# rusty-shell/rust-compress

Measured on AMD Instinct MI355X. Metric: GiB/s decoded output (batched blocks), higher is better.
Workload: dtype u8; 1 GPU; LZ4 block decode, 4096 independent 64 KiB blocks per GPU (BASELINE configs[1]); distribution=G-text, kernel_variant=0, parallelism=blocks sharded, 4096 per rank, no collective

## Files before the change

rust_compress_amd/csrc/k_lz4_decode_v8.hip:

```cpp
#include "rcx_dev.h"
#include "k_lz4_emit6.hip"

#ifndef RCX_V8_PSLEEP
#define RCX_V8_PSLEEP 16
#endif
#ifndef RCX_V8_ESLEEP
#define RCX_V8_ESLEEP 2
#endif
#ifndef RCX_FIELDS_ISA
#define RCX_FIELDS_ISA 1
#endif
#ifndef RCX_WALK_FORM
#define RCX_WALK_FORM 5
#endif
#ifndef RCX_V8_PRE
#define RCX_V8_PRE 128
#endif
#ifndef RCX_LINK_REPAIR
#define RCX_LINK_REPAIR 1
#endif
#ifndef RCX_WALK_STEPS
#define RCX_WALK_STEPS 16
#endif
#ifndef RCX_WALK_ISA_LOW
// ... 738 lines not shown
            const int agev = (agey ? 1 : 0) | ((RCX_AGE_LOW && (tail & 3u) < ((uint32_t)(RCX_AGE_LOW >> (4u * agerank)) & 15u)) ? 2 : 0);
            tail++;
            if (lane == 0) ring->tail = tail;
            if (X6 && plain6) { RCX_V8_STAT(10, lane == 0 && bt.why == B::SOLO_); RCX_V8_STAT(11, lane == 0 && bt.why == B::WIDE_); RCX_V8_STAT(12, lane == 0 ? (uint32_t)bt.ns : 0u); RCX_V8_STAT(13, lane == 0); }
            if (X6 && plain6 && this->emit6(bt.ns, w1, p0, agev)) {
                if (this->after_batch(bt, st)) break;
                continue;
            }
            RCX_V8_STAT(9, lane == 0 && bt.ns > 0);
            RCX_V8_STAT(10, lane == 0 && bt.why == B::SOLO_); RCX_V8_STAT(11, lane == 0 && bt.why == B::WIDE_); RCX_V8_STAT(12, lane == 0 ? (uint32_t)bt.ns : 0u); RCX_V8_STAT(13, lane == 0);
            const bool cont = (w1 & 0x80u) != 0;
            if (cont) w1 &= ~0xffu;
            const uint32_t L = w1 & 0xffu, M = (w1 >> 8) & 0xffu;
            const uint32_t hop = ((int)lane < bt.ns && !cont) ? 3u + L + (L >= 15u ? 1u : 0u) + (M >= 19u ? 1u : 0u) : 0u;
            const uint32_t w0 = p0 + rcx_wave_incl_scan(hop) - hop + 1u + (L >= 15u ? 1u : 0u);
            int lo = 0, e = 0;
            RCX_MARK("x8_pre_emit");
            if (PROF8) { const uint64_t t_ = (uint64_t)__builtin_readcyclecounter(); this->pw[1] += t_ - te1; te1 = t_; }
#if defined(RCX_DUMMY_SALU) || defined(RCX_DUMMY_VALU) || defined(RCX_DUMMY_VCMP) || defined(RCX_DUMMY_VCMPX) || defined(RCX_DUMMY_RL) || defined(RCX_DUMMY_SNOP) || defined(RCX_DUMMY_BR) || defined(RCX_DUMMY_LDS)
            {
                uint32_t ds_ = 0, dv_ = this->lane;
#ifdef RCX_DUMMY_SALU
#pragma unroll
                for (int k_ = 0; k_ < RCX_DUMMY_SALU; k_++) asm volatile("s_add_u32 %0, %0, 1" : "+s"(ds_) : : "scc");
#endif
#ifdef RCX_DUMMY_VALU
#pragma unroll
                for (int k_ = 0; k_ < RCX_DUMMY_VALU; k_++) asm volatile("v_add_u32_e32 %0, 1, %0" : "+v"(dv_));
#endif
#ifdef RCX_DUMMY_VCMP
#pragma unroll
                for (int k_ = 0; k_ < RCX_DUMMY_VCMP; k_++) asm volatile("v_cmp_lt_u32_e32 vcc, %0, %0" : : "v"(dv_) : "vcc");
#endif
#ifdef RCX_DUMMY_VCMPX
#pragma unroll
                for (int k_ = 0; k_ < RCX_DUMMY_VCMPX; k_++) asm volatile("v_cmpx_le_u32_e32 vcc, %0, %0" : : "v"(dv_) : "vcc");
#endif
#ifdef RCX_DUMMY_RL
#pragma unroll
                for (int k_ = 0; k_ < RCX_DUMMY_RL; k_++) asm volatile("v_readlane_b32 %0, %1, 0" : "=s"(ds_) : "v"(dv_));
#endif
#ifdef RCX_DUMMY_SNOP
#pragma unroll
                for (int k_ = 0; k_ < RCX_DUMMY_SNOP; k_++) asm volatile("s_nop 0");
#endif
#ifdef RCX_DUMMY_BR
#pragma unroll
                for (int k_ = 0; k_ < RCX_DUMMY_BR; k_++) asm volatile("s_cbranch_execz 1f\n1:");
#endif
#ifdef RCX_DUMMY_LDS
#pragma unroll
                for (int k_ = 0; k_ < RCX_DUMMY_LDS; k_++) asm volatile("ds_read_b32 %0, %1" : "=v"(dv_) : "v"(0u) : "memory");
                asm volatile("s_waitcnt lgkmcnt(0)" ::: "memory");
#endif
                asm volatile("" : : "s"(ds_), "v"(dv_));
            }
#endif
            if (CUT & 8) { if (!(CUT & 32)) this->oend += RCX_U(__builtin_amdgcn_readlane(w0, 63)) & 1u; lo = bt.ns; if (bt.why == B::END_ || bt.why == B::ERR_) break; continue; }
            while (lo < bt.ns && !e) e = this->template emit5<false, PRED, CUT, (SPLIT ? SPLIT : 64), typename std::conditional<X6, Lz4V8, void>::type>(bt.ns, lo, w0, w1, nullptr, agev);
            RCX_MARK("x8_post_emit");
            if (e) { st = e; break; }
            if (PROF8) te1 = (uint64_t)__builtin_readcyclecounter();
            if (this->after_batch(bt, st)) break;
            if (PROF8) this->pw[3] += (uint64_t)__builtin_readcyclecounter() - te1;
            RCX_MARK("x8_loop_end");
        }
        if (st && lane == 0) ring->abort_ = 1;
        if (RCX_AGE_DYN && lane == 0) __hip_atomic_store(prog + wslot, RCX_PROG_FIN, __ATOMIC_RELAXED, __HIP_MEMORY_SCOPE_AGENT);
        if (!st) this->flush(this->oend, true);
        *st_out = st;
        *len_out = st ? 0u : this->oend;
    }

    __device__ void run_parser8()
    {
        this->lane = rcx_lane();
        const unsigned lane = this->lane;
        const uint32_t n = this->n;
        const uint32_t inmis = (uint32_t)((uintptr_t)this->in & 15u);
        uint32_t head = 0;
        uint32_t c = 0;
        int32_t cs = -(int32_t)inmis;
        uint32_t lcnt = 0;
        while (c < n) {
            V8P_T0();
            if (RCX_V8_ADAPT) ring_prio(head, RCX_V8_LOW_WALK);
            else if (c != 0 && RCX_WALK_PRIO != RCX_PARSER_PRIO) __builtin_amdgcn_s_setprio(RCX_WALK_PRIO);
            else if ((RCX_AGE_PRIO & 16) && this->agey) __builtin_amdgcn_s_setprio(RCX_PARSER_PRIO + 1); else __builtin_amdgcn_s_setprio(RCX_PARSER_PRIO);
            stage8(cs);
#if RCX_V8_PREFETCH
            {
                const int64_t q = (int64_t)cs + CH + CSLACK + 64 * (int64_t)lane;
                if (q >= 0 && q + 4 <= (int64_t)n) { const uint32_t x = *(const rcx_u32_u*)(this->in + q); asm volatile("" : : "v"(x)); }
            }
#endif
            const int nseg = ((int64_t)n - cs >= CH) ? NSEG : (int)(((int64_t)n - cs + SEGB - 1) / SEGB);
            const int k0 = (int)(((int32_t)c - cs) / SEGB);
            const int32_t s = cs + SEGB * (int32_t)lane;
            const uint32_t e = ((int64_t)s + SEGB < (int64_t)n) ? (uint32_t)(s + SEGB) : n;
            const uint32_t nx = RCX_U(next_tok_c(c));
            const bool giant = nx >= n || (int64_t)nx >= (int64_t)cs + CH;
            const bool mine = !giant && (int)lane >= k0 && (int)lane < nseg;
            int32_t p0 = s - PRE; p0 = p0 < 0 ? 0 : p0;
            uint32_t p = ((int)lane == k0) ? c : (uint32_t)p0;
            uint64_t map = (giant && (int)lane == k0) ? 1ull << (c - (uint32_t)s) : 0ull;
            RCX_MARK("p8_walk");
#if (RCX_WALK_FORM == 5) && !defined(RCX_NO_WALK_ASM)
            if (n >= 20u) {
                const uint32_t adj = RCX_U((uint32_t)(uintptr_t)this->cbuf - (uint32_t)this->cbase);
                const uint32_t e20 = e < n - 19u ? e : n - 19u;
                const uint32_t ead = mine ? e20 + adj : 0u, sgad = (uint32_t)s + adj;
                uint32_t ad = p + adj;
                for (;;) {
                    uint32_t steps = RCX_WALK_STEPS;
                    const uint64_t slow = walk_steps2(ad, ead, sgad, map, steps);
                    if (PROF8) pp[7] += steps == 0xffffffffu ? 0 : RCX_WALK_STEPS - steps;
                    if (slow) { if (RCX_INV_BALLOT(slow)) ad = next_tok(ad - adj) + adj; }
                    else if (steps == 0xffffffffu) break;
                    if (RCX_V8_ADAPT) ring_prio(head, RCX_V8_LOW_WALK);
                }
                p = ad - adj; p = p < n ? p : n;
            }
#elif (RCX_WALK_FORM >= 2) && !defined(RCX_NO_WALK_ASM)
            if (n >= 20u && (RCX_WALK_FORM == 2 || head == 0 || (RCX_WALK_FORM == 4 && head - RCX_U(this->ring8->tail) < (uint32_t)RCX_WALK_ISA_LOW))) {
                uint32_t mlo = (uint32_t)map, mhi = (uint32_t)(map >> 32);
                const uint64_t minem = __ballot(mine);
                for (;;) {
                    uint32_t steps = 4;
                    const uint64_t slow = walk_steps(p, e, (uint32_t)s, mlo, mhi, minem, steps);
                    if (PROF8) pp[7] += steps == 0xffffffffu ? 0 : 4 - steps;
                    if (slow) { if (RCX_INV_BALLOT(slow)) p = next_tok(p); }
                    else if (steps == 0xffffffffu) break;
                    if (RCX_V8_ADAPT) ring_prio(head, RCX_V8_LOW_WALK);
                }
                map = (uint64_t)mlo | ((uint64_t)mhi << 32);
            } else
#endif
            for (uint32_t wstep = 0;; wstep++) {
                const bool go = mine && p < e;
                if (!__ballot(go)) break;
                if (PROF8) pp[7] += 1;
                if (RCX_V8_ADAPT && (wstep & 3u) == 3u) ring_prio(head, RCX_V8_LOW_WALK);
#if RCX_WALK_FORM == 0 || RCX_WALK_FORM >= 3
                if (go) {
                    if ((int32_t)p >= s) map |= 1ull << (p - (uint32_t)s);
                    p = next_tok_c(p);
                }
#else
                const uint32_t q = next_tok_c(p, go);
                const uint64_t bit = (go && (int32_t)p >= s) ? 1ull << ((p - (uint32_t)s) & 63u) : 0ull;
                map |= bit;
                p = go ? q : p;
#endif
            }
            RCX_MARK("p8_walk_end");
            const uint32_t ex = p;
            V8P_ADD(0);
            if (RCX_V8_ADAPT) ring_prio(head, RCX_V8_LOW_WALK);
            uint32_t lowv = 0; bool clr = false;
            if (giant) c = nx;
            else {
                const uint32_t eprev = (uint32_t)__shfl_up((int)ex, 1);
                const bool chk = mine && (int)lane > k0;
                bool ok = false;
                if (chk && eprev < e) { lowv = eprev - (uint32_t)s; ok = (map >> lowv) & 1ull; }
                if (!ok) lowv = 0;
                unsigned long long bad = __ballot(chk && !ok);
#ifdef RCX_LINK_NOREPAIR
                bad = 0;
#endif
                c = RCX_U(__builtin_amdgcn_readlane(ex, nseg - 1));
                int k = 0; uint32_t cin = 0; bool forced = false;
                for (;;) {
                    if (!forced) {
                        if (!bad) break;
                        k = __ffsll(bad) - 1;
                        cin = RCX_U(__builtin_amdgcn_readlane(ex, k - 1));
                    }
                    bad &= ~(1ull << k);
                    const uint32_t sk = (uint32_t)(cs + SEGB * k);
                    const uint32_t ek = (sk + SEGB < n) ? sk + SEGB : n;
                    const uint32_t exk = RCX_U(__builtin_amdgcn_readlane(ex, k));
                    uint32_t X;
                    if (cin >= ek) { if ((int)lane == k) { clr = true; lowv = 0; } X = cin; }
                    else {
                        const uint64_t mk = (uint64_t)RCX_U(__builtin_amdgcn_readlane((uint32_t)map, k)) | ((uint64_t)RCX_U(__builtin_amdgcn_readlane((uint32_t)(map >> 32), k)) << 32);
                        if ((mk >> (cin - sk)) & 1ull) { if ((int)lane == k) { lowv = cin - sk; clr = false; } X = exk; }
                        else {
                            if (PROF8) pp[8] += 1;
                            uint64_t tm = 0;
                            uint32_t q = cin;
#if RCX_LINK_REPAIR
                            {
                                const int32_t qi = (int32_t)(sk + lane) - this->cbase;
                                const uint32_t t = ((const RCX_LDS_AS uint8_t*)this->cbuf)[qi];
                                const uint32_t L = t >> 4;
                                const uint32_t x = ((const RCX_LDS_AS uint8_t*)this->cbuf)[qi + 3 + (int32_t)L];
                                const bool ext = (t & 15u) == 15u;
                                const bool fastp = n >= 20u && sk + lane <= n - 20u && L != 15u && !(ext && x == 255u);
                                const uint32_t dv = fastp ? (ext ? 4u : 3u) + L : 128u;
                                uint32_t rel = cin - sk;
                                RCX_V8_STAT(7, lane == 0);
                                for (;;) {
                                    uint64_t vis = 0;
                                    RCX_HOP_WALK(dv, rel, vis);
                                    tm |= vis;
                                    RCX_V8_STAT(7, lane == 0 ? (uint64_t)__popcll(vis) << 32 : 0ull); RCX_V8_STAT(19, lane == 0 && rel >= 128u);
                                    if (rel < 128u) { q = sk + rel; break; }
                                    q = RCX_U(next_tok_c(sk + rel - 128u));
                                    if (q >= ek) break;
                                    rel = q - sk;
                                }
                            }
                            if ((int)lane == k) { map = tm; lowv = 0; clr = false; }
                            X = q;
#else
                            while (q < ek && !((mk >> (q - sk)) & 1ull)) { tm |= 1ull << (q - sk); q = RCX_U(next_tok_c(q)); }
                            const bool merged = q < ek;
                            const uint64_t nm = (merged ? mk & ~((1ull << (q - sk)) - 1ull) : 0ull) | tm;
                            if ((int)lane == k) { map = nm; lowv = 0; clr = false; }
                            X = merged ? exk : q;
#endif
                        }
                    }
                    if (k == nseg - 1) c = X;
                    forced = X != exk && k + 1 < nseg;
                    if (forced) { k++; cin = X; }
                }
            }
            if (clr) map = 0;
            map &= ~((1ull << lowv) - 1ull);
            if (!mine && !giant) map = 0;
            V8P_ADD(1);
            RCX_MARK("p8_link_end");
            if (PROF8) pp[6] += 1;
            const int nwin = (nseg + LWIN - 1) / LWIN;
            for (int w = k0 / LWIN; w < nwin; w++) {
                if (RCX_V8_ADAPT) ring_prio(head);
                const int sl = LWIN * w + (int)(lane >> 3);
                const uint32_t mlo = (uint32_t)__builtin_amdgcn_ds_bpermute(sl << 2, (int)(uint32_t)map);
                const uint32_t mhi = (uint32_t)__builtin_amdgcn_ds_bpermute(sl << 2, (int)(uint32_t)(map >> 32));
                uint32_t bits = (((lane & 4u) ? mhi : mlo) >> (8u * (lane & 3u))) & 0xffu;
                if (sl >= nseg) bits = 0;
                const uint32_t cnt = (uint32_t)__popc(bits);
                const uint32_t incl = rcx_wave_incl_scan(cnt);
                uint32_t at = lcnt + incl - cnt;
                const int32_t bpos = SEGB * sl + 8 * (int32_t)(lane & 7u);
                for (;;) {
                    if (!__ballot(bits != 0)) break;
                    if (bits) { const uint32_t b = (uint32_t)__ffs(bits) - 1u; bits &= bits - 1u; list[at++] = (int16_t)(bpos + (int32_t)b); }
                }
                lcnt += RCX_U(__builtin_amdgcn_readlane(incl, 63));
                rcx_wave_sync();
                V8P_ADD(2);
                RCX_MARK("p8_list_end");
                const bool last = (w + 1 == nwin) && c >= n;
                uint32_t pos = 0;
                while (lcnt - pos >= 64u || (last && lcnt > pos)) {
                    const int used = batch8(head, cs, pos, lcnt - pos < 64u ? lcnt - pos : 64u);
                    if (used < 0) return;
                    pos += (uint32_t)used;
                    if (PROF8) t0_ = (uint64_t)__builtin_readcyclecounter();
                }
                if (pos) {
                    const uint32_t left = lcnt - pos;
                    const int16_t v = lane < left ? list[pos + lane] : (int16_t)0;
                    rcx_wave_sync();
                    if (lane < left) list[lane] = v;
                    lcnt = left;
                    rcx_wave_sync();
                }
            }
            int32_t ncs = cs + CH;
            if (c < n && (int64_t)c >= (int64_t)ncs + CH) ncs = (int32_t)((c + inmis) & ~15u) - (int32_t)inmis;
            if (lcnt) {
                if ((int32_t)(int16_t)RCX_U((uint32_t)(uint16_t)list[0]) - (ncs - cs) < -30000) {
                    uint32_t pos = 0;
                    while (lcnt > pos) { const int used = batch8(head, cs, pos, lcnt - pos); if (used < 0) return; pos += (uint32_t)used; }
                    lcnt = 0;
                } else {
                    if (lane < lcnt) list[lane] = (int16_t)(list[lane] - (int16_t)(ncs - cs));
                    rcx_wave_sync();
                }
            }
            cs = ncs;
        }
        post(head, 0, B::END_, 0, 0, 0, 0, 0, 0, false, 0, 0, 0);
    }
};

template <int TC = 1024, int HH = 768, bool PROF8 = false, int PRE_ = RCX_V8_PRE, int SPLIT_ = 32, bool PRED = false, int PRR = 2, int CUT = 0, bool MIRROR = false, int X6_ = -1>
__global__ __launch_bounds__(128, 8) void k_lz4_decode_v8(rcx_kargs a, int only_status = 0)
{
    constexpr bool X6 = RCX_X6_MODE != 0 && (X6_ < 0 ? (CUT == 0 && !PRED && SPLIT_ != 0 && !MIRROR) : X6_ != 0);
    typedef Lz4V8<TC, HH, X6 ? 0 : 16, PROF8, PRE_, SPLIT_, PRED, PRR, CUT, MIRROR, X6> S;
    __shared__ __align__(16) uint32_t s_mtab[X6 ? 20 * RCX_X6_MROW : 4];
    const uint64_t tk0 = PROF8 ? (uint64_t)__builtin_readcyclecounter() : 0;
    const uint64_t rt0 = PROF8 ? (uint64_t)__builtin_amdgcn_s_memrealtime() : 0;
    __shared__ __align__(16) uint8_t s_wbuf[S::WBUF5 + 16 + (X6 ? 16 : 0)];
    __shared__ __align__(16) typename S::Ring8 s_ring;
    __shared__ __align__(16) uint8_t s_cbuf[S::CBUF8 + 16];
    __shared__ int16_t s_list[S::LISTN];
    __shared__ uint32_t s_lmap[64];
    const uint32_t b = blockIdx.x;
    if (b >= a.nblocks) return;
    if (only_status && a.status[b] != only_status) return;
    if (MIRROR && a.gate) {
        uint32_t r = 0;
#pragma unroll
        for (int i = 0; i < 15; i++) r += b >= a.gate_bnd[i] ? 1u : 0u;
        if (r || a.gate_all) {
            if (threadIdx.x == 0) {
                const uint64_t t0 = __builtin_amdgcn_s_memrealtime();
                uint32_t ok = 1;
                if (b == (r ? a.gate_bnd[r - 1] : 0u)) {
                    while (__hip_atomic_load(a.gate_host + r, __ATOMIC_RELAXED, __HIP_MEMORY_SCOPE_SYSTEM) != a.gate_seq) {
                        __builtin_amdgcn_s_sleep(60);
                        if (__builtin_amdgcn_s_memrealtime() - t0 > (uint64_t)a.gate_ticks) { ok = 0; break; }
                    }
                    if (ok) __hip_atomic_store(a.gate + r, a.gate_seq, __ATOMIC_RELEASE, __HIP_MEMORY_SCOPE_SYSTEM);
                }
                while (ok && __hip_atomic_load(a.gate + r, __ATOMIC_RELAXED, __HIP_MEMORY_SCOPE_SYSTEM) != a.gate_seq) {
                    __builtin_amdgcn_s_sleep(127); __builtin_amdgcn_s_sleep(127);
                    if (__builtin_amdgcn_s_memrealtime() - t0 > (uint64_t)a.gate_ticks) ok = 0;
                }
                s_lmap[0] = ok;
            }
            __syncthreads();
            const uint32_t ok = s_lmap[0];
            __builtin_amdgcn_fence(__ATOMIC_ACQUIRE, "");
            __syncthreads();
            if (!ok) { if (threadIdx.x == 0) a.status[b] = (int32_t)RCX_ST_GATE; return; }
        }
    }
    if (threadIdx.x == 0) { RCX_LDS_AS typename S::Ring8* r0 = (RCX_LDS_AS typename S::Ring8*)&s_ring; r0->head = 0; r0->tail = 0; r0->abort_ = 0; }
    __syncthreads();
    const uint32_t role = (uint32_t)__builtin_amdgcn_readfirstlane((int)(threadIdx.x >> 6));
    S s;
    s.in = a.in_base + a.in_off[b];
    s.n = (uint32_t)a.in_len[b];
    s.out = a.out_base + a.out_off[b];
    if (MIRROR) s.out2 = a.out_mirror + a.out_off[b];
    const uint64_t cap64 = a.out_cap[b];
    s.cap = cap64 > 0xffffffffull ? 0xffffffffu : (uint32_t)cap64;
    s.cbuf = s_cbuf;
    s.wb_ = s_wbuf + (X6 ? 16 : 0);
    s.epos = nullptr;
    s.ring = nullptr;
    s.ring8 = (RCX_LDS_AS typename S::Ring8*)&s_ring;
    s.list = s_list;
    s.lmap = s_lmap;
    s.mtab = (RCX_LDS_AS uint32_t*)s_mtab;
    if (RCX_AGE_DYN) {
        const uint32_t hw = (uint32_t)__builtin_amdgcn_s_getreg((15 << 11) | (0 << 6) | 4);
        const uint32_t xcc = (uint32_t)__builtin_amdgcn_s_getreg((3 << 11) | (0 << 6) | 20) & 15u;
        s.prog = g_lz4_prog + 8u * (((hw >> 4) & 0xfffu) | (xcc << 12));
        s.wslot = hw & 7u;
    }
    if (role == 0) {
        if (RCX_AGE_DYN && (threadIdx.x & 63u) == 0) __hip_atomic_store(s.prog + s.wslot, RCX_PROG_PARSER, __ATOMIC_RELAXED, __HIP_MEMORY_SCOPE_AGENT);
        if (RCX_AGE_PRIO & 16) s.agey = (((uint32_t)__builtin_amdgcn_s_getreg((3 << 11) | (0 << 6) | 4) >> 1) & 7u) >= (uint32_t)RCX_AGE_SPLIT;
        s.run_parser8();
        if (PROF8 && a.scratch && (threadIdx.x & 63u) == 0) {
            uint64_t* q = (uint64_t*)a.scratch + (size_t)b * 32;
            for (int i = 0; i < 10; i++) q[i] = s.pp[i];
            q[10] = (uint64_t)__builtin_readcyclecounter() - tk0;
        }
        return;
    }
    int32_t st; uint32_t olen;
    const uint32_t hwid = (PROF8 || RCX_AGE_PRIO) ? (uint32_t)__builtin_amdgcn_s_getreg((3 << 11) | (0 << 6) | 4) : 0u;
    s.agey = RCX_AGE_PRIO ? ((hwid >> 1) & 7u) >= (uint32_t)RCX_AGE_SPLIT : true;
    s.agerank = (hwid >> 1) & 3u;
    RCX_SETPRIO_EXEC(s.agey);
    if (X6) { s.lane = rcx_lane(); s.mtab_init(); }
    s.run_executor8(&st, &olen);
    if (PROF8 && a.scratch && (threadIdx.x & 63u) == 0) {
        uint64_t* q = (uint64_t*)a.scratch + (size_t)b * 32;
        q[11] = (uint64_t)__builtin_readcyclecounter() - tk0;
        q[12] = hwid;
        q[13] = rt0; q[14] = (uint64_t)__builtin_amdgcn_s_memrealtime();
        q[15] = (uint64_t)(uint32_t)__builtin_amdgcn_s_getreg((31 << 11) | (0 << 6) | 4) | ((uint64_t)(uint32_t)__builtin_amdgcn_s_getreg((31 << 11) | (0 << 6) | 20) << 32);
        for (int i = 0; i < 12; i++) q[16 + i] = s.pw[i];
    }
    if ((threadIdx.x & 63u) == 0) {
        a.status[b] = st;
        a.out_len[b] = olen;
        if (a.in_used) a.in_used[b] = s.n;
    }
}
```

rust_compress_amd/csrc/k_lz4_emit6.hip:

```cpp
#pragma once
#include "rcx_dev.h"

#ifndef RCX_X6_MROW
#define RCX_X6_MROW 9
#endif
#ifndef RCX_X6_RR
#define RCX_X6_RR 3
#endif
#ifndef RCX_X6_MODE
#define RCX_X6_MODE 1
#endif
#ifndef RCX_X6_ROUNDS_ASM
#define RCX_X6_ROUNDS_ASM 1
#endif
#ifndef RCX_X6_EARLY
#define RCX_X6_EARLY 1
#endif
#ifndef RCX_V8_STAT
#define RCX_V8_STAT(slot, v) ((void)0)
#endif

#if !defined(RCX_NO_ROUNDS_ASM) && !defined(RCX_NO_MSKOR_ASM)
__device__ __forceinline__ uint64_t rcx_lz4_rounds6(uint32_t s0, uint32_t d4, uint32_t mc, uint32_t dep_lo, uint32_t dep_hi, uint64_t pend, uint32_t tb, uint32_t fix)
{
    uint32_t t0, t1, nv, sa, sh, da, r0, r1, r2, r3, r4, r5, m0, m1, m2, m3, m4, prog = 0;
    uint64_t sT, sF;
    asm volatile(
        "s_mov_b64 vcc, %[pend]\n\t"
        "L_top_%=:\n\t"
        "v_and_b32_e32 %[t0], vcc_lo, %[dlo]\n\t"
        "v_and_b32_e32 %[t1], vcc_hi, %[dhi]\n\t"
        "v_or_b32_e32 %[t0], %[t0], %[t1]\n\t"
        "v_cmp_eq_u32_e64 %[sT], 0, %[t0]\n\t"
        "s_and_b64 exec, %[sT], vcc\n\t"
        "s_cbranch_scc0 L_out_%=\n\t"
        "v_add_u32_e32 %[sa], %[s0], %[prog]\n\t"
        "v_sub_u32_e32 %[nv], %[mc], %[prog]\n\t"
        "v_and_b32_e32 %[t0], -4, %[sa]\n\t"
        "ds_read_b32 %[r0], %[t0]\n\t"
        "ds_read_b32 %[r1], %[t0] offset:4\n\t"
        "ds_read_b32 %[r2], %[t0] offset:8\n\t"
        "ds_read_b32 %[r3], %[t0] offset:12\n\t"
        "ds_read_b32 %[r4], %[t0] offset:16\n\t"
        "ds_read_b32 %[r5], %[t0] offset:20\n\t"
        "v_min_u32_e32 %[nv], 16, %[nv]\n\t"
        "v_mad_u32_u24 %[t1], %[nv], %[mrow], %[tb]\n\t"
        "ds_read_b32 %[m0], %[t1]\n\t"
        "ds_read_b32 %[m1], %[t1] offset:4\n\t"
        "ds_read_b32 %[m2], %[t1] offset:8\n\t"
        "ds_read_b32 %[m3], %[t1] offset:12\n\t"
        "ds_read_b32 %[m4], %[t1] offset:16\n\t"
        "v_and_b32_e32 %[sh], 3, %[sa]\n\t"
        "v_add_u32_e32 %[da], %[d4], %[prog]\n\t"
        "v_add_u32_e32 %[prog], %[prog], %[nv]\n\t"
        "v_cmp_ge_u32_e64 %[sF], %[prog], %[mc]\n\t"
        "s_waitcnt lgkmcnt(9)\n\t"
        "v_alignbyte_b32 %[r0], %[r1], %[r0], %[sh]\n\t"
        "s_waitcnt lgkmcnt(8)\n\t"
        "v_alignbyte_b32 %[r1], %[r2], %[r1], %[sh]\n\t"
        "s_waitcnt lgkmcnt(7)\n\t"
        "v_alignbyte_b32 %[r2], %[r3], %[r2], %[sh]\n\t"
        "s_waitcnt lgkmcnt(6)\n\t"
        "v_alignbyte_b32 %[r3], %[r4], %[r3], %[sh]\n\t"
        "s_waitcnt lgkmcnt(5)\n\t"
        "v_alignbyte_b32 %[r4], %[r5], %[r4], %[sh]\n\t"
        "s_waitcnt lgkmcnt(4)\n\t"
        "v_and_b32_e32 %[m0], %[m0], %[fix]\n\t"
        "v_and_b32_e32 %[r0], %[r0], %[m0]\n\t"
        "ds_mskor_b32 %[da], %[m0], %[r0]\n\t"
        "s_waitcnt lgkmcnt(4)\n\t"
        "v_and_b32_e32 %[r1], %[r1], %[m1]\n\t"
        "ds_mskor_b32 %[da], %[m1], %[r1] offset:4\n\t"
        "s_waitcnt lgkmcnt(4)\n\t"
        "v_and_b32_e32 %[r2], %[r2], %[m2]\n\t"
        "ds_mskor_b32 %[da], %[m2], %[r2] offset:8\n\t"
        "s_waitcnt lgkmcnt(4)\n\t"
        "v_and_b32_e32 %[r3], %[r3], %[m3]\n\t"
        "ds_mskor_b32 %[da], %[m3], %[r3] offset:12\n\t"
        "s_waitcnt lgkmcnt(4)\n\t"
        "v_and_b32_e32 %[r4], %[r4], %[m4]\n\t"
        "ds_mskor_b32 %[da], %[m4], %[r4] offset:16\n\t"
        "s_mov_b64 exec, -1\n\t"
        "s_andn2_b64 vcc, vcc, %[sF]\n\t"
        "s_cbranch_scc1 L_top_%=\n\t"
        "L_out_%=:\n\t"
        "s_mov_b64 exec, -1\n\t"
        "s_mov_b64 %[pend], vcc\n\t"
        : [pend] "+s"(pend), [prog] "+v"(prog), [t0] "=&v"(t0), [t1] "=&v"(t1), [nv] "=&v"(nv), [sa] "=&v"(sa), [sh] "=&v"(sh), [da] "=&v"(da),
          [r0] "=&v"(r0), [r1] "=&v"(r1), [r2] "=&v"(r2), [r3] "=&v"(r3), [r4] "=&v"(r4), [r5] "=&v"(r5),
          [m0] "=&v"(m0), [m1] "=&v"(m1), [m2] "=&v"(m2), [m3] "=&v"(m3), [m4] "=&v"(m4), [sT] "=&s"(sT), [sF] "=&s"(sF)
        : [s0] "v"(s0), [d4] "v"(d4), [mc] "v"(mc), [dlo] "v"(dep_lo), [dhi] "v"(dep_hi), [tb] "v"(tb), [fix] "v"(fix), [mrow] "s"(4u * (uint32_t)RCX_X6_MROW)
        : "vcc", "scc", "memory");
    return pend;
}
#define RCX_HAVE_ROUNDS6 1
#endif

template <class Base, bool PROF8>
struct Lz4X6 : Base {
    typedef Base P5;
    typedef typename Base::B B;
    RCX_LDS_AS uint32_t* mtab = nullptr;

    __device__ __forceinline__ void mtab_init()
    {
        for (uint32_t i = this->lane; i < 20u * (uint32_t)RCX_X6_MROW; i += 64u) {
            const int32_t e = (int32_t)(i / (uint32_t)RCX_X6_MROW), k = (int32_t)(i % (uint32_t)RCX_X6_MROW);
            int32_t t = e - 4 * k; t = t < 0 ? 0 : t > 4 ? 4 : t;
            mtab[i] = (k < 5 && t) ? (0xffffffffu >> (8 * (4 - t))) : 0u;
        }
        rcx_wave_sync();
    }
    template <int NW>
    __device__ __forceinline__ void store_frame(uint8_t* fp, uint32_t w0, uint32_t w1, uint32_t w2, uint32_t w3, uint32_t w4, uint32_t a, uint32_t n)
    {
#ifdef RCX_NO_MSKOR_ASM
        const uint32_t w[5] = {w0, w1, w2, w3, w4};
        for (uint32_t j = a; j < a + n; j++) fp[j] = (uint8_t)(w[j >> 2] >> (8u * (j & 3u)));
#else
        const RCX_LDS_AS uint32_t* te = mtab + (uint32_t)RCX_X6_MROW * (a + n);
#if RCX_X6_MROW == 8
        const rcx_u32x4 mv = *(const RCX_LDS_AS rcx_u32x4*)te;
#else
        rcx_u32x4 mv; mv[0] = te[0]; mv[1] = te[1]; mv[2] = te[2]; mv[3] = te[3];
#endif
        const uint32_t m0 = mv[0] & (0xffffffffu << (8u * a));
        const uint32_t fa = (uint32_t)(uintptr_t)fp;
        if (NW >= 5) {
            const uint32_t m4 = te[4];
            asm volatile("ds_mskor_b32 %0, %1, %2\n\tds_mskor_b32 %0, %3, %4 offset:4\n\tds_mskor_b32 %0, %5, %6 offset:8\n\tds_mskor_b32 %0, %7, %8 offset:12\n\tds_mskor_b32 %0, %9, %10 offset:16"
                         :: "v"(fa), "v"(m0), "v"(w0 & m0), "v"(mv[1]), "v"(w1 & mv[1]), "v"(mv[2]), "v"(w2 & mv[2]), "v"(mv[3]), "v"(w3 & mv[3]), "v"(m4), "v"(w4 & m4) : "memory");
        } else {
            asm volatile("ds_mskor_b32 %0, %1, %2\n\tds_mskor_b32 %0, %3, %4 offset:4\n\tds_mskor_b32 %0, %5, %6 offset:8\n\tds_mskor_b32 %0, %7, %8 offset:12"
                         :: "v"(fa), "v"(m0), "v"(w0 & m0), "v"(mv[1]), "v"(w1 & mv[1]), "v"(mv[2]), "v"(w2 & mv[2]), "v"(mv[3]), "v"(w3 & mv[3]) : "memory");
        }
#endif
    }

    __device__ __forceinline__ bool emit6(int ns, uint32_t w1raw, uint32_t p0, int young)
    {
        const unsigned lane = this->lane;
        const uint8_t* in = this->in; uint8_t* out = this->out; uint8_t* wb_ = this->wb_;
        const uint32_t cap = this->cap, n = this->n;
        uint64_t tq_ = PROF8 ? (uint64_t)__builtin_readcyclecounter() : 0;
#define X6P_ADD(slot) do { RCX_MARK("emit6_" #slot); if (PROF8) { const uint64_t t1_ = (uint64_t)__builtin_readcyclecounter(); this->pw[slot] += t1_ - tq_; tq_ = t1_; } } while (0)
        this->make_room(B::TCAP);
        X6P_ADD(11);
        const uint32_t oend0 = this->oend;
        const uint32_t w1 = (int)lane < ns ? w1raw : 0u;
        const uint32_t L = w1 & 0x7fu, M = (w1 >> 8) & 0xffu, off = w1 >> 16;
        const uint32_t lx = L >= 15u ? 1u : 0u;
        const uint32_t hop = ((int)lane < ns && !(w1 & 0x80u)) ? 3u + L + lx + (M >= 19u ? 1u : 0u) : 0u;
        const uint32_t len = L + M;
        const uint32_t sc = rcx_wave_incl_scan(len | (hop << 16));
        const uint32_t T = RCX_U(__builtin_amdgcn_readlane(sc, 63)) & 0xffffu;
        if (T > (uint32_t)B::TCAP || cap - oend0 < T + 64u) return false;
        const uint32_t lincl = sc & 0xffffu;
        const uint32_t ostart = oend0 + lincl - len;
        const uint32_t mdst = ostart + L;
        const uint32_t src = p0 + (sc >> 16) - hop + 1u + lx;
        const uint32_t slo = mdst - off;
        const uint32_t re = this->rlo_eff();
        const bool isfar = slo < re;
        if (__ballot(off > mdst || (isfar && slo < 4u))) return false;
        X6P_ADD(4);

        const int32_t lbase = this->lbase;
        const int32_t li_o = (int32_t)ostart - lbase, li_m = li_o + (int32_t)L;
        const uint32_t a1 = (uint32_t)li_o & 3u, a2 = (uint32_t)li_m & 3u;
        uint32_t ql = src - a1; { const uint32_t qm = n - 36u; ql = ql < qm ? ql : qm; }
        const bool lit2 = __ballot(L > 16u) != 0;
        const rcx_u32x4 g0 = *(const rcx_u32x4_u*)(in + ql);
        const rcx_u32x4 g1 = *(const rcx_u32x4_u*)(in + ql + 16);
        uint32_t g2 = 0;
        if (lit2) g2 = *(const rcx_u32_u*)(in + ql + 32);
        rcx_u32x4 f0, f1; uint32_t f2;
        RCX_NOINIT4(f0); RCX_NOINIT4(f1); f2 = 0;
#ifndef RCX_X6_NOFAR
        if (re) {
#else
        if (false) {
#endif
            const uint32_t qf = isfar ? slo - a2 : 0u;
            f0 = *(const rcx_u32x4_u*)(out + qf);
            f1 = *(const rcx_u32x4_u*)(out + qf + 16);
            f2 = *(const rcx_u32_u*)(out + qf + 32);
        }
        RCX_SETPRIO_ROUND(young);

        const uint32_t shi = (slo + M < mdst) ? slo + M : mdst;
        bool inb = M != 0u && !isfar && shi > oend0;
        uint32_t S = off;
        uint32_t ka, kb;
        {
            uint32_t* const lmap = this->lmap;
            uint8_t* const lcnt = (uint8_t*)(lmap + P5::LMW);
            lmap[lane] = 0;
            rcx_wave_sync();
            const uint32_t rel = lincl - len;
            atomicOr(&lmap[rel >> 5], 1u << (rel & 31u));
            rcx_wave_sync();
            const uint32_t pc = (uint32_t)__popc(lmap[lane]);
            const uint32_t ex = rcx_wave_incl_scan(pc) - pc;
            lcnt[lane] = (uint8_t)ex;
            rcx_wave_sync();
            int32_t ra = (int32_t)(slo - oend0), rb = (int32_t)(shi - oend0) - 1;
            ra = ra > 0 ? ra : 0; rb = rb > 0 ? rb : 0;
            uint32_t ca = lcnt[ra >> 5], ma = lmap[ra >> 5], cb2 = lcnt[rb >> 5], mb = lmap[rb >> 5];
            RCX_SETTLE4(ca, ma, cb2, mb);
            ka = (ca + (uint32_t)__popc(ma & (0xffffffffu >> (31u - ((uint32_t)ra & 31u)))) - 1u) & 63u;
            kb = (cb2 + (uint32_t)__popc(mb & (0xffffffffu >> (31u - ((uint32_t)rb & 31u)))) - 1u) & 63u;
        }
        unsigned long long dep = 0;
        {
            const uint32_t pmd = (uint32_t)__builtin_amdgcn_ds_bpermute((int)(ka << 2), (int)((isfar || off < M) ? 0xffffffffu : mdst));
            const uint32_t prod = (inb && ka == kb && slo >= pmd && off >= M) ? ka : 64u;
            RCX_V8_STAT(28, inb && ka != kb); RCX_V8_STAT(29, inb && ka == kb && slo < pmd); RCX_V8_STAT(30, inb && ka == kb && slo >= pmd && off < M);
            RCX_V8_STAT(31, inb && ka == kb && shi <= pmd && pmd != 0xffffffffu);
            uint32_t st = prod | (ka << 7) | (kb << 13) | ((uint32_t)inb << 19);
#pragma unroll
            for (int rr = 0; rr < RCX_X6_RR; rr++) {
                const bool has = (st & 64u) == 0u;
                const uint32_t j = has ? (st & 63u) : lane;
                const uint32_t Sj = (uint32_t)__builtin_amdgcn_ds_bpermute((int)(j << 2), (int)S);
                const uint32_t pk = (uint32_t)__builtin_amdgcn_ds_bpermute((int)(j << 2), (int)st);
                const uint32_t Sn = S + Sj;
                const bool ok = has && mdst - Sn >= re && Sn <= mdst;
                S = ok ? Sn : S;
                st = ok ? pk : (st | 64u);
            }
            ka = (st >> 7) & 63u; kb = (st >> 13) & 63u; inb = (st >> 19) & 1u;
            const unsigned long long upto = (kb >= 63) ? ~0ull : ((2ull << kb) - 1ull);
            dep = inb ? (upto & ~((1ull << ka) - 1ull) & ((1ull << lane) - 1ull)) : 0ull;
        }

        X6P_ADD(5);
        {
            const uint32_t n1 = L < 16u ? L : 16u;
            uint8_t* fp = wb_ + (li_o - (int32_t)a1);
            if (n1) store_frame<5>(fp, g0[0], g0[1], g0[2], g0[3], g1[0], a1, n1);
            if (lit2) { if (L > 16u) store_frame<5>(fp + 16, g1[0], g1[1], g1[2], g1[3], g2, a1, L - n1); }
        }
#if RCX_X6_EARLY
        const bool early = M != 0u && !isfar && !inb && off >= M && (RCX_X6_EARLY == 1 || M <= 16u);
        RCX_V8_STAT(15, early);
        if (early) {
            const int32_t sb = (int32_t)(mdst - S) - lbase - (int32_t)a2;
#ifdef RCX_NO_MSKOR_ASM
            const RCX_LDS_AS uint32_t* q = (const RCX_LDS_AS uint32_t*)(wb_ + (sb & ~3));
#else
            uint32_t qa = (uint32_t)(uintptr_t)wb_ + (uint32_t)(sb & ~3);
            asm volatile("" : "+v"(qa));
            const RCX_LDS_AS uint32_t* q = (const RCX_LDS_AS uint32_t*)qa;
#endif
            const uint32_t sh = (uint32_t)sb & 3u;
            const uint32_t r0 = q[0], r1 = q[1], r2 = q[2], r3 = q[3], r4 = q[4], r5 = q[5];
            f0[0] = RCX_ALIGNBYTE(r1, r0, sh); f0[1] = RCX_ALIGNBYTE(r2, r1, sh); f0[2] = RCX_ALIGNBYTE(r3, r2, sh); f0[3] = RCX_ALIGNBYTE(r4, r3, sh);
            f1[0] = RCX_ALIGNBYTE(r5, r4, sh);
            if (RCX_X6_EARLY == 1 && M > 16u) {
                const uint32_t r6 = q[6], r7 = q[7], r8 = q[8], r9 = q[9];
                f1[1] = RCX_ALIGNBYTE(r6, r5, sh); f1[2] = RCX_ALIGNBYTE(r7, r6, sh); f1[3] = RCX_ALIGNBYTE(r8, r7, sh); f2 = RCX_ALIGNBYTE(r9, r8, sh);
            }
        }
        const uint32_t mf = (isfar || early) ? M : 0u;
        if (__ballot(mf != 0u)) {
#else
        const uint32_t mf = isfar ? M : 0u;
        if (re) {
#endif
            const uint32_t n1 = mf < 16u ? mf : 16u;
            uint8_t* fp = wb_ + (li_m - (int32_t)a2);
            if (n1) store_frame<5>(fp, f0[0], f0[1], f0[2], f0[3], f1[0], a2, n1);
            if (mf > 16u) store_frame<5>(fp + 16, f1[0], f1[1], f1[2], f1[3], f2, a2, mf - n1);
        }
        rcx_wave_sync();
        X6P_ADD(6);

        {
            const int32_t dfr = li_m - (int32_t)a2;
            const bool ovl = M != 0u && off < 16u && off < M;
            const int32_t sfr = isfar ? dfr : (int32_t)(mdst - S) - lbase - (int32_t)a2;
            const uint32_t Mc = mf ? 0u : M;
            auto fill_run = [&]() __attribute__((always_inline)) {
                uint32_t done = 0, back = off;
                while (done < M) {
                    uint32_t c = back < M - done ? back : M - done;
                    c = c < 16u ? c : 16u;
                    const int32_t d = li_m + (int32_t)done;
                    const uint32_t ar = (uint32_t)d & 3u;
                    const int32_t sb = d - (int32_t)back - (int32_t)ar;
                    const uint32_t* q = (const uint32_t*)(wb_ + (sb & ~3));
                    const uint32_t sh = (uint32_t)sb & 3u;
                    const uint32_t r0 = q[0], r1 = q[1], r2 = q[2], r3 = q[3], r4 = q[4], r5 = q[5];
                    store_frame<5>(wb_ + (d - (int32_t)ar), RCX_ALIGNBYTE(r1, r0, sh), RCX_ALIGNBYTE(r2, r1, sh), RCX_ALIGNBYTE(r3, r2, sh),
                                   RCX_ALIGNBYTE(r4, r3, sh), RCX_ALIGNBYTE(r5, r4, sh), ar, c);
                    done += c;
                    if (2u * back <= off + done) back *= 2u;
                }
            };
            unsigned long long pm = __ballot(Mc != 0u);
#ifdef RCX_HAVE_ROUNDS6
            if (RCX_X6_ROUNDS_ASM) {
                const uint32_t wa = (uint32_t)(uintptr_t)wb_;
                const unsigned long long depx = dep | (ovl ? 1ull << lane : 0ull);
                while (pm) {
                    pm = rcx_lz4_rounds6(wa + (uint32_t)sfr, wa + (uint32_t)dfr, Mc, (uint32_t)depx, (uint32_t)(depx >> 32), pm,
                                         (uint32_t)(uintptr_t)mtab + a2 * (4u * (uint32_t)RCX_X6_MROW), 0xffffffffu << (8u * a2));
                    if (!pm) break;
                    const bool fill = ovl && ((pm >> lane) & 1ull) && (pm & dep) == 0ull;
                    if (fill) fill_run();
                    rcx_wave_sync();
                    pm &= ~__ballot(fill);
                }
            } else
#endif
            {
            uint32_t prog = 0;
            RCX_V8_STAT(16, Mc != 0u); RCX_V8_STAT(17, Mc != 0u && dep != 0ull); RCX_V8_STAT(18, Mc > 16u);
            uint32_t nr_ = 0;
            while (pm) {
                nr_++; RCX_V8_STAT(14, lane == 0);
                const bool ready = ((pm >> lane) & 1ull) && (pm & dep) == 0ull;
                const bool fill = ready && ovl;
                const uint32_t left = Mc - prog;
                const uint32_t nv = (ready && !ovl) ? (left < 16u ? left : 16u) : 0u;
                const int32_t sb = sfr + (int32_t)prog;
                const uint32_t* q = (const uint32_t*)(wb_ + (sb & ~3));
                const uint32_t sh = (uint32_t)sb & 3u;
                uint32_t r0 = 0, r1 = 0, r2 = 0, r3 = 0, r4 = 0, r5 = 0;
                if (nv) { r0 = q[0]; r1 = q[1]; r2 = q[2]; r3 = q[3]; r4 = q[4]; r5 = q[5]; }
                rcx_wave_sync();
                if (nv) store_frame<5>(wb_ + (dfr + (int32_t)prog), RCX_ALIGNBYTE(r1, r0, sh), RCX_ALIGNBYTE(r2, r1, sh), RCX_ALIGNBYTE(r3, r2, sh),
                               RCX_ALIGNBYTE(r4, r3, sh), RCX_ALIGNBYTE(r5, r4, sh), a2, nv);
                if (fill) fill_run();
                rcx_wave_sync();
                prog += fill ? Mc : nv;
                pm = __ballot(prog < Mc);
            }
            RCX_V8_STAT(20 + (nr_ < 7u ? nr_ : 7u), lane == 0);
            }
        }
        X6P_ADD(7);
        RCX_SETPRIO_FLUSH(young);
        this->oend = RCX_U(oend0 + T);
        this->flush(this->oend, false);
        if (RCX_FLUSH_PRIO != RCX_EXEC_PRIO) RCX_SETPRIO_EXEC(young);
        X6P_ADD(8);
        if (PROF8) this->pw[10] += 1;
#undef X6P_ADD
        RCX_V8_STAT(8, lane == 0);
        return true;
    }
};
```

Baseline: 582.2 GiB/s.

## Widen mask rows and pair LDS reads; skip empty fifth-word masked stores

Raises the mask-table row stride to 12 words so each row's first four masks load with one ds_read_b128, and pairs source reads via ds_read2_b32, cutting the number of LDS instructions per copy round. The inline-asm rounds loop now uses fixed VGPRs (v44-v53) with recomputed waitcnt values. Store-frame calls skip the fifth ds_mskor when no lane in the wave writes past 16 bytes, found with a wave ballot. The wider mask table uses more LDS, and a static_assert is added to keep LDS use within the budget for sixteen workgroups per CU. Hard-coded registers may constrain the register allocator.

```diff
diff --git a/rust_compress_amd/csrc/k_lz4_decode_v8.hip b/rust_compress_amd/csrc/k_lz4_decode_v8.hip
--- a/rust_compress_amd/csrc/k_lz4_decode_v8.hip
+++ b/rust_compress_amd/csrc/k_lz4_decode_v8.hip
@@ -1064,6 +1064,9 @@
     __shared__ __align__(16) uint8_t s_cbuf[S::CBUF8 + 16];
     __shared__ int16_t s_list[S::LISTN];
     __shared__ uint32_t s_lmap[64];
+    static_assert(!(X6 && TC == 1024 && HH == 768 && !PROF8 && RCX_X6_MODE == 1) ||
+                  ((sizeof(s_mtab) + 15) & ~15u) + ((sizeof(s_wbuf) + 15) & ~15u) + ((sizeof(s_ring) + 15) & ~15u) + ((sizeof(s_cbuf) + 15) & ~15u) +
+                  ((sizeof(s_list) + 15) & ~15u) + sizeof(s_lmap) <= 10240, "k_lz4_decode_v8: more LDS than sixteen workgroups a CU allow");
     const uint32_t b = blockIdx.x;
     if (b >= a.nblocks) return;
     if (only_status && a.status[b] != only_status) return;
diff --git a/rust_compress_amd/csrc/k_lz4_emit6.hip b/rust_compress_amd/csrc/k_lz4_emit6.hip
--- a/rust_compress_amd/csrc/k_lz4_emit6.hip
+++ b/rust_compress_amd/csrc/k_lz4_emit6.hip
@@ -2,7 +2,14 @@
 #include "rcx_dev.h"
 
 #ifndef RCX_X6_MROW
-#define RCX_X6_MROW 9
+#define RCX_X6_MROW 12
+#endif
+#define RCX_X6_MROW_WIDE ((RCX_X6_MROW) % 4 == 0)
+#ifndef RCX_X6_NW4
+#define RCX_X6_NW4 3
+#endif
+#ifndef RCX_X6_PAIR
+#define RCX_X6_PAIR 1
 #endif
 #ifndef RCX_X6_RR
 #define RCX_X6_RR 3
@@ -19,11 +26,45 @@
 #ifndef RCX_V8_STAT
 #define RCX_V8_STAT(slot, v) ((void)0)
 #endif
+#ifdef RCX_X6_FRAME_STATS
+inline unsigned long long g_x6_frame_stat[4];
+extern "C" __attribute__((used, visibility("default"))) inline unsigned long long* rcx_x6_frame_stats() { return g_x6_frame_stat; }
+#define RCX_X6_STAT(slot, v) (g_x6_frame_stat[slot] += (unsigned long long)(v))
+#else
+#define RCX_X6_STAT(slot, v) ((void)0)
+#endif
 
 #if !defined(RCX_NO_ROUNDS_ASM) && !defined(RCX_NO_MSKOR_ASM)
+#define RCX_R6_S0 "v48"
+#define RCX_R6_S1 "v49"
+#define RCX_R6_S2 "v50"
+#define RCX_R6_S3 "v51"
+#define RCX_R6_S4 "v52"
+#define RCX_R6_S5 "v53"
+#define RCX_R6_M0 "v44"
+#define RCX_R6_M1 "v45"
+#define RCX_R6_M2 "v46"
+#define RCX_R6_M3 "v47"
+#if RCX_X6_PAIR
+#define RCX_R6_SRC_READS "ds_read2_b32 v[48:49], %[t0] offset1:1\n\tds_read2_b32 v[50:51], %[t0] offset0:2 offset1:3\n\tds_read2_b32 v[52:53], %[t0] offset0:4 offset1:5\n\t"
+#define RCX_R6_NSRC 3
+#else
+#define RCX_R6_SRC_READS "ds_read_b32 v48, %[t0]\n\tds_read_b32 v49, %[t0] offset:4\n\tds_read_b32 v50, %[t0] offset:8\n\tds_read_b32 v51, %[t0] offset:12\n\tds_read_b32 v52, %[t0] offset:16\n\tds_read_b32 v53, %[t0] offset:20\n\t"
+#define RCX_R6_NSRC 6
+#endif
+#if RCX_X6_MROW_WIDE
+#define RCX_R6_ROW_READS "ds_read_b128 v[44:47], %[t1]\n\tds_read_b32 %[m4], %[t1] offset:16\n\t"
+#define RCX_R6_NROW 2
+#elif RCX_X6_PAIR
+#define RCX_R6_ROW_READS "ds_read2_b32 v[44:45], %[t1] offset1:1\n\tds_read2_b32 v[46:47], %[t1] offset0:2 offset1:3\n\tds_read_b32 %[m4], %[t1] offset:16\n\t"
+#define RCX_R6_NROW 3
+#else
+#define RCX_R6_ROW_READS "ds_read_b32 v44, %[t1]\n\tds_read_b32 v45, %[t1] offset:4\n\tds_read_b32 v46, %[t1] offset:8\n\tds_read_b32 v47, %[t1] offset:12\n\tds_read_b32 %[m4], %[t1] offset:16\n\t"
+#define RCX_R6_NROW 5
+#endif
 __device__ __forceinline__ uint64_t rcx_lz4_rounds6(uint32_t s0, uint32_t d4, uint32_t mc, uint32_t dep_lo, uint32_t dep_hi, uint64_t pend, uint32_t tb, uint32_t fix)
 {
-    uint32_t t0, t1, nv, sa, sh, da, r0, r1, r2, r3, r4, r5, m0, m1, m2, m3, m4, prog = 0;
+    uint32_t t0, t1, nv, sa, sh, da, m4, prog = 0;
     uint64_t sT, sF;
     asm volatile(
         "s_mov_b64 vcc, %[pend]\n\t"
@@ -37,49 +78,63 @@
         "v_add_u32_e32 %[sa], %[s0], %[prog]\n\t"
         "v_sub_u32_e32 %[nv], %[mc], %[prog]\n\t"
         "v_and_b32_e32 %[t0], -4, %[sa]\n\t"
-        "ds_read_b32 %[r0], %[t0]\n\t"
-        "ds_read_b32 %[r1], %[t0] offset:4\n\t"
-        "ds_read_b32 %[r2], %[t0] offset:8\n\t"
-        "ds_read_b32 %[r3], %[t0] offset:12\n\t"
-        "ds_read_b32 %[r4], %[t0] offset:16\n\t"
-        "ds_read_b32 %[r5], %[t0] offset:20\n\t"
+        RCX_R6_SRC_READS
         "v_min_u32_e32 %[nv], 16, %[nv]\n\t"
         "v_mad_u32_u24 %[t1], %[nv], %[mrow], %[tb]\n\t"
-        "ds_read_b32 %[m0], %[t1]\n\t"
-        "ds_read_b32 %[m1], %[t1] offset:4\n\t"
-        "ds_read_b32 %[m2], %[t1] offset:8\n\t"
-        "ds_read_b32 %[m3], %[t1] offset:12\n\t"
-        "ds_read_b32 %[m4], %[t1] offset:16\n\t"
+        RCX_R6_ROW_READS
         "v_and_b32_e32 %[sh], 3, %[sa]\n\t"
         "v_add_u32_e32 %[da], %[d4], %[prog]\n\t"
         "v_add_u32_e32 %[prog], %[prog], %[nv]\n\t"
         "v_cmp_ge_u32_e64 %[sF], %[prog], %[mc]\n\t"
-        "s_waitcnt lgkmcnt(9)\n\t"
-        "v_alignbyte_b32 %[r0], %[r1], %[r0], %[sh]\n\t"
-        "s_waitcnt lgkmcnt(8)\n\t"
-        "v_alignbyte_b32 %[r1], %[r2], %[r1], %[sh]\n\t"
-        "s_waitcnt lgkmcnt(7)\n\t"
-        "v_alignbyte_b32 %[r2], %[r3], %[r2], %[sh]\n\t"
-        "s_waitcnt lgkmcnt(6)\n\t"
-        "v_alignbyte_b32 %[r3], %[r4], %[r3], %[sh]\n\t"
-        "s_waitcnt lgkmcnt(5)\n\t"
-        "v_alignbyte_b32 %[r4], %[r5], %[r4], %[sh]\n\t"
+#if RCX_X6_PAIR
+        "s_waitcnt lgkmcnt(%c[w0])\n\t"
+        "v_alignbyte_b32 " RCX_R6_S0 ", " RCX_R6_S1 ", " RCX_R6_S0 ", %[sh]\n\t"
+        "s_waitcnt lgkmcnt(%c[w1])\n\t"
+        "v_alignbyte_b32 " RCX_R6_S1 ", " RCX_R6_S2 ", " RCX_R6_S1 ", %[sh]\n\t"
+        "v_alignbyte_b32 " RCX_R6_S2 ", " RCX_R6_S3 ", " RCX_R6_S2 ", %[sh]\n\t"
+        "s_waitcnt lgkmcnt(%c[w2])\n\t"
+        "v_alignbyte_b32 " RCX_R6_S3 ", " RCX_R6_S4 ", " RCX_R6_S3 ", %[sh]\n\t"
+        "v_alignbyte_b32 " RCX_R6_S4 ", " RCX_R6_S5 ", " RCX_R6_S4 ", %[sh]\n\t"
+#else
+        "s_waitcnt lgkmcnt(%c[w0])\n\t"
+        "v_alignbyte_b32 " RCX_R6_S0 ", " RCX_R6_S1 ", " RCX_R6_S0 ", %[sh]\n\t"
+        "s_waitcnt lgkmcnt(%c[w0b])\n\t"
+        "v_alignbyte_b32 " RCX_R6_S1 ", " RCX_R6_S2 ", " RCX_R6_S1 ", %[sh]\n\t"
+        "s_waitcnt lgkmcnt(%c[w0c])\n\t"
+        "v_alignbyte_b32 " RCX_R6_S2 ", " RCX_R6_S3 ", " RCX_R6_S2 ", %[sh]\n\t"
+        "s_waitcnt lgkmcnt(%c[w0d])\n\t"
+        "v_alignbyte_b32 " RCX_R6_S3 ", " RCX_R6_S4 ", " RCX_R6_S3 ", %[sh]\n\t"
+        "s_waitcnt lgkmcnt(%c[w0e])\n\t"
+        "v_alignbyte_b32 " RCX_R6_S4 ", " RCX_R6_S5 ", " RCX_R6_S4 ", %[sh]\n\t"
+#endif
+        "s_waitcnt lgkmcnt(%c[wm])\n\t"
+        "v_and_b32_e32 " RCX_R6_M0 ", " RCX_R6_M0 ", %[fix]\n\t"
+        "v_and_b32_e32 " RCX_R6_S0 ", " RCX_R6_S0 ", " RCX_R6_M0 "\n\t"
+        "ds_mskor_b32 %[da], " RCX_R6_M0 ", " RCX_R6_S0 "\n\t"
+#if !RCX_X6_MROW_WIDE && !RCX_X6_PAIR
         "s_waitcnt lgkmcnt(4)\n\t"
-        "v_and_b32_e32 %[m0], %[m0], %[fix]\n\t"
-        "v_and_b32_e32 %[r0], %[r0], %[m0]\n\t"
-        "ds_mskor_b32 %[da], %[m0], %[r0]\n\t"
+#endif
+        "v_and_b32_e32 " RCX_R6_S1 ", " RCX_R6_S1 ", " RCX_R6_M1 "\n\t"
+        "ds_mskor_b32 %[da], " RCX_R6_M1 ", " RCX_R6_S1 " offset:4\n\t"
+#if !RCX_X6_MROW_WIDE
+        "s_waitcnt lgkmcnt(%c[wm2])\n\t"
+#endif
+        "v_and_b32_e32 " RCX_R6_S2 ", " RCX_R6_S2 ", " RCX_R6_M2 "\n\t"
+        "ds_mskor_b32 %[da], " RCX_R6_M2 ", " RCX_R6_S2 " offset:8\n\t"
+#if !RCX_X6_MROW_WIDE && !RCX_X6_PAIR
         "s_waitcnt lgkmcnt(4)\n\t"
-        "v_and_b32_e32 %[r1], %[r1], %[m1]\n\t"
-        "ds_mskor_b32 %[da], %[m1], %[r1] offset:4\n\t"
+#endif
+        "v_and_b32_e32 " RCX_R6_S3 ", " RCX_R6_S3 ", " RCX_R6_M3 "\n\t"
+        "ds_mskor_b32 %[da], " RCX_R6_M3 ", " RCX_R6_S3 " offset:12\n\t"
         "s_waitcnt lgkmcnt(4)\n\t"
-        "v_and_b32_e32 %[r2], %[r2], %[m2]\n\t"
-        "ds_mskor_b32 %[da], %[m2], %[r2] offset:8\n\t"
-        "s_waitcnt lgkmcnt(4)\n\t"
-        "v_and_b32_e32 %[r3], %[r3], %[m3]\n\t"
-        "ds_mskor_b32 %[da], %[m3], %[r3] offset:12\n\t"
-        "s_waitcnt lgkmcnt(4)\n\t"
-        "v_and_b32_e32 %[r4], %[r4], %[m4]\n\t"
-        "ds_mskor_b32 %[da], %[m4], %[r4] offset:16\n\t"
+#if RCX_X6_NW4 & 1
+        "v_cmp_ne_u32_e64 %[sT], 0, %[m4]\n\t"
+        "s_cmp_eq_u64 %[sT], 0\n\t"
+        "s_cbranch_scc1 L_four_%=\n\t"
+#endif
+        "v_and_b32_e32 " RCX_R6_S4 ", " RCX_R6_S4 ", %[m4]\n\t"
+        "ds_mskor_b32 %[da], %[m4], " RCX_R6_S4 " offset:16\n\t"
+        "L_four_%=:\n\t"
         "s_mov_b64 exec, -1\n\t"
         "s_andn2_b64 vcc, vcc, %[sF]\n\t"
         "s_cbranch_scc1 L_top_%=\n\t"
@@ -87,10 +142,12 @@
         "s_mov_b64 exec, -1\n\t"
         "s_mov_b64 %[pend], vcc\n\t"
         : [pend] "+s"(pend), [prog] "+v"(prog), [t0] "=&v"(t0), [t1] "=&v"(t1), [nv] "=&v"(nv), [sa] "=&v"(sa), [sh] "=&v"(sh), [da] "=&v"(da),
-          [r0] "=&v"(r0), [r1] "=&v"(r1), [r2] "=&v"(r2), [r3] "=&v"(r3), [r4] "=&v"(r4), [r5] "=&v"(r5),
-          [m0] "=&v"(m0), [m1] "=&v"(m1), [m2] "=&v"(m2), [m3] "=&v"(m3), [m4] "=&v"(m4), [sT] "=&s"(sT), [sF] "=&s"(sF)
-        : [s0] "v"(s0), [d4] "v"(d4), [mc] "v"(mc), [dlo] "v"(dep_lo), [dhi] "v"(dep_hi), [tb] "v"(tb), [fix] "v"(fix), [mrow] "s"(4u * (uint32_t)RCX_X6_MROW)
-        : "vcc", "scc", "memory");
+          [m4] "=&v"(m4), [sT] "=&s"(sT), [sF] "=&s"(sF)
+        : [s0] "v"(s0), [d4] "v"(d4), [mc] "v"(mc), [dlo] "v"(dep_lo), [dhi] "v"(dep_hi), [tb] "v"(tb), [fix] "v"(fix), [mrow] "s"(4u * (uint32_t)RCX_X6_MROW),
+          [w0] "n"(RCX_R6_NSRC + RCX_R6_NROW - (RCX_X6_PAIR ? 1 : 2)), [w1] "n"(RCX_R6_NSRC + RCX_R6_NROW - 2), [w2] "n"(RCX_R6_NSRC + RCX_R6_NROW - 3),
+          [wm] "n"(RCX_R6_NROW - 1), [wm2] "n"(RCX_X6_PAIR ? 3 : 4),
+          [w0b] "n"(RCX_R6_NSRC + RCX_R6_NROW - 3), [w0c] "n"(RCX_R6_NSRC + RCX_R6_NROW - 4), [w0d] "n"(RCX_R6_NSRC + RCX_R6_NROW - 5), [w0e] "n"(RCX_R6_NSRC + RCX_R6_NROW - 6)
+        : "vcc", "scc", "memory", "v44", "v45", "v46", "v47", "v48", "v49", "v50", "v51", "v52", "v53");
     return pend;
 }
 #define RCX_HAVE_ROUNDS6 1
@@ -112,21 +169,26 @@
         rcx_wave_sync();
     }
     template <int NW>
-    __device__ __forceinline__ void store_frame(uint8_t* fp, uint32_t w0, uint32_t w1, uint32_t w2, uint32_t w3, uint32_t w4, uint32_t a, uint32_t n)
+    __device__ __forceinline__ void store_frame(uint8_t* fp, uint32_t w0, uint32_t w1, uint32_t w2, uint32_t w3, uint32_t w4, uint32_t a, uint32_t n, unsigned long long any5 = ~0ull)
     {
 #ifdef RCX_NO_MSKOR_ASM
         const uint32_t w[5] = {w0, w1, w2, w3, w4};
-        for (uint32_t j = a; j < a + n; j++) fp[j] = (uint8_t)(w[j >> 2] >> (8u * (j & 3u)));
+        for (uint32_t j = a; j < a + n && j < (NW ? 4u * (uint32_t)NW : any5 ? 20u : 16u); j++) fp[j] = (uint8_t)(w[j >> 2] >> (8u * (j & 3u)));
 #else
         const RCX_LDS_AS uint32_t* te = mtab + (uint32_t)RCX_X6_MROW * (a + n);
-#if RCX_X6_MROW == 8
+#if RCX_X6_MROW_WIDE
         const rcx_u32x4 mv = *(const RCX_LDS_AS rcx_u32x4*)te;
 #else
         rcx_u32x4 mv; mv[0] = te[0]; mv[1] = te[1]; mv[2] = te[2]; mv[3] = te[3];
 #endif
         const uint32_t m0 = mv[0] & (0xffffffffu << (8u * a));
         const uint32_t fa = (uint32_t)(uintptr_t)fp;
-        if (NW >= 5) {
+        if (NW == 0) {
+            const uint32_t m4 = te[4];
+            asm volatile("ds_mskor_b32 %0, %1, %2\n\tds_mskor_b32 %0, %3, %4 offset:4\n\tds_mskor_b32 %0, %5, %6 offset:8\n\tds_mskor_b32 %0, %7, %8 offset:12\n\t"
+                         "s_cmp_eq_u64 %11, 0\n\ts_cbranch_scc1 L_f4_%=\n\tds_mskor_b32 %0, %9, %10 offset:16\n\tL_f4_%=:"
+                         :: "v"(fa), "v"(m0), "v"(w0 & m0), "v"(mv[1]), "v"(w1 & mv[1]), "v"(mv[2]), "v"(w2 & mv[2]), "v"(mv[3]), "v"(w3 & mv[3]), "v"(m4), "v"(w4 & m4), "s"(any5) : "memory", "scc");
+        } else if (NW >= 5) {
             const uint32_t m4 = te[4];
             asm volatile("ds_mskor_b32 %0, %1, %2\n\tds_mskor_b32 %0, %3, %4 offset:4\n\tds_mskor_b32 %0, %5, %6 offset:8\n\tds_mskor_b32 %0, %7, %8 offset:12\n\tds_mskor_b32 %0, %9, %10 offset:16"
                          :: "v"(fa), "v"(m0), "v"(w0 & m0), "v"(mv[1]), "v"(w1 & mv[1]), "v"(mv[2]), "v"(w2 & mv[2]), "v"(mv[3]), "v"(w3 & mv[3]), "v"(m4), "v"(w4 & m4) : "memory");
@@ -135,6 +197,16 @@
                          :: "v"(fa), "v"(m0), "v"(w0 & m0), "v"(mv[1]), "v"(w1 & mv[1]), "v"(mv[2]), "v"(w2 & mv[2]), "v"(mv[3]), "v"(w3 & mv[3]) : "memory");
         }
 #endif
+    }
+
+    __device__ __forceinline__ void store_frame_w(uint8_t* fp, uint32_t w0, uint32_t w1, uint32_t w2, uint32_t w3, uint32_t w4, uint32_t a, uint32_t n)
+    {
+        const unsigned long long any5 = (RCX_X6_NW4 & 2) ? __ballot(n != 0u && a + n > 16u) : ~0ull;
+#ifdef RCX_X6_FRAME_STATS
+        { const bool any = __ballot(n != 0u) != 0, none5 = __ballot(n != 0u && a + n > 16u) == 0;
+          RCX_X6_STAT(0, this->lane == 0 && any); RCX_X6_STAT(1, this->lane == 0 && any && none5); }
+#endif
+        if (n) store_frame<(RCX_X6_NW4 & 2) ? 0 : 5>(fp, w0, w1, w2, w3, w4, a, n, any5);
     }
 
     __device__ __forceinline__ bool emit6(int ns, uint32_t w1raw, uint32_t p0, int young)
@@ -238,12 +310,12 @@
         {
             const uint32_t n1 = L < 16u ? L : 16u;
             uint8_t* fp = wb_ + (li_o - (int32_t)a1);
-            if (n1) store_frame<5>(fp, g0[0], g0[1], g0[2], g0[3], g1[0], a1, n1);
-            if (lit2) { if (L > 16u) store_frame<5>(fp + 16, g1[0], g1[1], g1[2], g1[3], g2, a1, L - n1); }
+            store_frame_w(fp, g0[0], g0[1], g0[2], g0[3], g1[0], a1, n1);
+            if (lit2) store_frame_w(fp + 16, g1[0], g1[1], g1[2], g1[3], g2, a1, L - n1);
         }
 #if RCX_X6_EARLY
         const bool early = M != 0u && !isfar && !inb && off >= M && (RCX_X6_EARLY == 1 || M <= 16u);
-        RCX_V8_STAT(15, early);
+        RCX_V8_STAT(15, early); RCX_X6_STAT(2, M != 0u && isfar);
         if (early) {
             const int32_t sb = (int32_t)(mdst - S) - lbase - (int32_t)a2;
 #ifdef RCX_NO_MSKOR_ASM
@@ -270,8 +342,8 @@
 #endif
             const uint32_t n1 = mf < 16u ? mf : 16u;
             uint8_t* fp = wb_ + (li_m - (int32_t)a2);
-            if (n1) store_frame<5>(fp, f0[0], f0[1], f0[2], f0[3], f1[0], a2, n1);
-            if (mf > 16u) store_frame<5>(fp + 16, f1[0], f1[1], f1[2], f1[3], f2, a2, mf - n1);
+            store_frame_w(fp, f0[0], f0[1], f0[2], f0[3], f1[0], a2, n1);
+            if (__ballot(mf > 16u)) store_frame_w(fp + 16, f1[0], f1[1], f1[2], f1[3], f2, a2, mf - n1);
         }
         rcx_wave_sync();
         X6P_ADD(6);
@@ -330,8 +402,8 @@
                 uint32_t r0 = 0, r1 = 0, r2 = 0, r3 = 0, r4 = 0, r5 = 0;
                 if (nv) { r0 = q[0]; r1 = q[1]; r2 = q[2]; r3 = q[3]; r4 = q[4]; r5 = q[5]; }
                 rcx_wave_sync();
-                if (nv) store_frame<5>(wb_ + (dfr + (int32_t)prog), RCX_ALIGNBYTE(r1, r0, sh), RCX_ALIGNBYTE(r2, r1, sh), RCX_ALIGNBYTE(r3, r2, sh),
-                               RCX_ALIGNBYTE(r4, r3, sh), RCX_ALIGNBYTE(r5, r4, sh), a2, nv);
+                store_frame_w(wb_ + (dfr + (int32_t)prog), RCX_ALIGNBYTE(r1, r0, sh), RCX_ALIGNBYTE(r2, r1, sh), RCX_ALIGNBYTE(r3, r2, sh),
+                              RCX_ALIGNBYTE(r4, r3, sh), RCX_ALIGNBYTE(r5, r4, sh), a2, nv);
                 if (fill) fill_run();
                 rcx_wave_sync();
                 prog += fill ? Mc : nv;
```

New measurement: 599.5 GiB/s (median of 6 runs). +3.0%, better.
